# ndmarco/BayesFMMM

Hardware: AMD Instinct MI355X
Metric: Gibbs iterations/sec (whole node) at n_funct=4096, K=3, P=30 (higher is better)
Workload: dtype f64; 1 GPU; BFMMM_warm_start sweep, n_funct=4096, n_i=100, K=3, P=30, M=6, fp64, one independent chain per GPU (1 chain(s): a chain does not shard, replicas only); chains=1, chains_per_gpu=1

## Files before the change

bayesfmmm_amd/_lib.py:

```python
import ctypes as C
import os

_HERE = os.path.dirname(os.path.abspath(__file__))
LIB_PATH = os.environ.get("BFMMM_LIB_PATH", os.path.join(_HERE, "libbfmmm_hip.so"))

c_double_p = C.POINTER(C.c_double)
c_int64_p = C.POINTER(C.c_int64)


class BfmmmConfig(C.Structure):
    _fields_ = [("model", C.c_int32), ("n_funct", C.c_int32), ("K", C.c_int32), ("n_eigen", C.c_int32),
                ("basis_degree", C.c_int32), ("n_internal_knots", C.c_int32), ("P", C.c_int32),
                ("tot_mcmc_iters", C.c_int32), ("c", C.c_double * 8), ("b", C.c_double), ("nu_1", C.c_double),
                ("alpha1l", C.c_double), ("alpha2l", C.c_double), ("beta1l", C.c_double), ("beta2l", C.c_double),
                ("a_Z_PM", C.c_double), ("a_pi_PM", C.c_double), ("var_alpha3", C.c_double),
                ("var_epsilon1", C.c_double), ("var_epsilon2", C.c_double), ("alpha_nu", C.c_double),
                ("beta_nu", C.c_double), ("alpha_eta", C.c_double), ("beta_eta", C.c_double),
                ("alpha_0", C.c_double), ("beta_0", C.c_double)]


SYMBOLS = {
    "bfmmm_config_defaults": (None, [C.POINTER(BfmmmConfig)]),
    "bfmmm_create": (C.c_int, [C.POINTER(BfmmmConfig), C.c_int, c_double_p, c_double_p, c_int64_p, c_double_p,
                               c_double_p, C.POINTER(C.c_void_p)]),
    "bfmmm_destroy": (None, [C.c_void_p]),
    "bfmmm_create_batch": (C.c_int, [C.POINTER(BfmmmConfig), C.c_int, c_double_p, c_double_p, c_int64_p, c_double_p,
                                     c_double_p, C.c_int, C.POINTER(C.c_void_p)]),
    "bfmmm_create_from_basis_batch": (C.c_int, [C.POINTER(BfmmmConfig), C.c_int, c_double_p, c_double_p, c_int64_p, C.c_int,
                                                C.c_int, c_double_p, C.c_int, C.c_int, C.POINTER(C.c_void_p)]),
    "bfmmm_select_chain": (C.c_int, [C.c_void_p, C.c_int]),
    "bfmmm_n_chains": (C.c_int, [C.c_void_p]),
    "bfmmm_set_chain_id_stride": (C.c_int, [C.c_void_p, C.c_uint32]),
    "bfmmm_gather_best": (C.c_int, [C.POINTER(C.c_void_p), C.c_int, c_double_p, C.POINTER(C.c_int32), C.POINTER(C.c_int)]),
    "bfmmm_set_covariates": (C.c_int, [C.c_void_p, c_double_p, C.c_int, C.c_int]),
    "bfmmm_get_basis": (C.c_int, [C.c_void_p, c_double_p, C.c_int64]),
    "bfmmm_set_state": (C.c_int, [C.c_void_p, C.c_char_p, c_double_p, C.c_int64]),
    "bfmmm_get_state": (C.c_int, [C.c_void_p, C.c_char_p, c_double_p, C.c_int64]),
    "bfmmm_init_state": (C.c_int, [C.c_void_p, C.c_int, C.c_uint64, C.c_uint32]),
    "bfmmm_run": (C.c_int, [C.c_void_p, C.c_uint32, C.c_int, C.c_int, C.c_uint64, C.c_uint32, C.c_int, C.c_double]),
    "bfmmm_prepare_run": (C.c_int, [C.c_void_p, C.c_uint32, C.c_int, C.c_int, C.c_uint64, C.c_uint32, C.c_int]),
    "bfmmm_set_slot_base": (C.c_int, [C.c_void_p, C.c_int]),
    "bfmmm_create_from_basis": (C.c_int, [C.POINTER(BfmmmConfig), C.c_int, c_double_p, c_double_p, c_int64_p, C.c_int, C.c_int,
                                          c_double_p, C.c_int, C.POINTER(C.c_void_p)]),
    "bfmmm_tempered_transition": (C.c_int, [C.c_void_p, C.c_uint32, C.c_int, C.c_int, C.c_double, C.c_uint64, C.c_uint32,
                                            c_double_p, C.POINTER(C.c_int)]),
    "bfmmm_get_chain": (C.c_int, [C.c_void_p, C.c_char_p, C.c_int, c_double_p, C.c_int64]),
    "bfmmm_chain_diagnostics": (C.c_int, [C.c_void_p, C.c_char_p, C.c_int, C.c_int, C.c_int64, c_double_p, c_double_p, c_double_p,
                                          c_double_p, c_double_p, c_double_p, c_double_p, C.c_int64]),
    "bfmmm_debug_get": (C.c_int, [C.c_void_p, C.c_char_p, c_double_p, C.c_int64, c_int64_p]),
    "bfmmm_set_profile": (C.c_int, [C.c_void_p, C.c_int]),
    "bfmmm_get_timing": (C.c_int, [C.c_void_p, C.c_char_p, C.POINTER(C.c_double), c_int64_p]),
    "bfmmm_set_exact_instances": (None, [C.c_int]),
    "bfmmm_set_solo_pair_gram": (None, [C.c_int]),
    "bfmmm_last_error": (C.c_char_p, []),
}

_LIB = None


def load():
    global _LIB
    if _LIB is None:
        if not os.path.exists(LIB_PATH):
            raise RuntimeError(
                f"{LIB_PATH} is missing: build it with `python -c 'import __graft_entry__ as g; g.build()'` "
                "(hipcc --offload-arch=gfx950). bayesfmmm_amd has no CPU fallback.")
        lib = C.CDLL(LIB_PATH)
        for name, (res, args) in SYMBOLS.items():
            fn = getattr(lib, name)
            fn.restype = res
            fn.argtypes = args
        _LIB = lib
    return _LIB


class BfmmmError(RuntimeError):
    pass


def check(rc):
    if rc != 0:
        raise BfmmmError(load().bfmmm_last_error().decode())
```

bayesfmmm_amd/csrc/bfmmm_capi.hip:

```cpp
#include "../../include/bfmmm.h"
#include "model.hpp"
#include "rng.hpp"

#include <algorithm>
#include <cmath>
#include <cstdio>
#include <cstring>
#include <map>
#include <chrono>
#include <mutex>
#include <string>
#include <tuple>
#include <vector>

namespace bfmmm {
int launch_stats_functional(int degree, int n, int P, int LREC, const int64_t* off, const double* t, const double* y,
                            const double* knots, int n_knots, double* rec, int* ni, double* B_dense, int* err,
                            hipStream_t st);
void launch_stats_multivariate(int n, int P, int LREC, const double* Y, double* rec, int* ni, hipStream_t st);
void launch_stats_totals(int n, int LREC, int yy_off, const double* rec, const int* ni, double* out_yy,
                         long long* out_counts, hipStream_t st);
int launch_curve(const Ctx& c, int which, int do_update, hipStream_t st);
int curve_blocks(int n, int P);
void prepare_curve_kernels();
void prepare_sweep_kernels();
void launch_pair_gram(const Ctx& c, int do_pg, int NKS, int KS, hipStream_t st);
int pair_gram_body(const Ctx& c, int KS, int& G);
size_t pair_gram_lds_bytes(const Dims& d, int KS);
void launch_pg_reduce(const Ctx& c, int NKS, hipStream_t st);
bool pgp_geometry(const Dims& d, int nch, int KS, int NKS, PgPack& g);
size_t pgp_pack_doubles(const PgPack& g);
void launch_pair_gram_pack(const Ctx& c, const PgPack& g, double* pack, hipStream_t st);
void launch_factor(const Ctx& c, hipStream_t st);
int launch_sweep(const Ctx& c, hipStream_t st);
void launch_sweep_tables(const Ctx& c, hipStream_t st);
size_t sweep_tab_ints(int A);
void launch_loglik(const Ctx& c, int use_rss_part, int r_stored, hipStream_t st);
void launch_loglik_flush(const Ctx& c, hipStream_t st, uint32_t* status_out);
void launch_fill_slots(const Ctx& c, double* chain, const double* cur, size_t len, int s0, int s1, hipStream_t st);
void launch_cov_block(const Ctx& c, hipStream_t st);
int cov_step_blocks(int nblk_curve);
int cov_w2_chunks(int n);
void prepare_cov_kernels();
bool cov_block_fits(const Ctx& c);
#ifdef BFMMM_TIMELINE
void fetch_wgtrace(unsigned long long* out);
void fetch_ztrace(unsigned long long* out);
void fetch_zphase(unsigned long long* out);
void fetch_fct(unsigned long long* out);
#endif
}

using namespace bfmmm;

static thread_local std::string g_err;
static constexpr int GRAPH_UNROLL = 10;
static std::mutex g_capture_mutex;
static int fail(const std::string& msg) { g_err = msg; return 1; }

#define HIPCHK(x)                                                                                   \
// ... 10 lines not shown
enum { FAM_TOTAL = 0, FAM_Z, FAM_PG, FAM_FACTOR, FAM_SWEEP, FAM_CHI, FAM_LOGLIK, FAM_REDUCE, FAM_COUNT };
static const char* kFamNames[FAM_COUNT] = {"total", "curve_z", "pair_gram", "factor", "sweep", "curve_chi", "loglik", "pg_reduce"};

struct bfmmm_handle {
  bfmmm_config cfg;
  int device = 0;
  hipStream_t st = nullptr;
  hipEvent_t evA = nullptr;
  Ctx c;
  int nch = 1;
  int sel = 0;
  int T = 0;
  int64_t n_obs = 0;
  double* d_t = nullptr; double* d_y = nullptr; int64_t* d_off = nullptr; double* d_knots = nullptr; int n_knots = 0;
  std::vector<void*> allocs;
  char* arena = nullptr;
  char* arena_cov = nullptr;
  uint32_t* status_host = nullptr;
  uint32_t* status_dev = nullptr;
  size_t pg_part_doubles = 0;
  static constexpr int MAX_SUB = 4;
  char* dry_snap = nullptr;
  size_t dry_snap_bytes = 0;
  double* pg_pack[MAX_SUB + 1] = {};
  size_t pg_pack_doubles[MAX_SUB + 1] = {};
  hipStream_t sub_st[MAX_SUB] = {nullptr, nullptr, nullptr, nullptr};
  hipEvent_t sub_ev[MAX_SUB] = {nullptr, nullptr, nullptr, nullptr};
  struct CachedGraph { int sub, kind, reps; hipGraphExec_t g; };
  std::vector<CachedGraph> graphs;
  using GraphKey = std::tuple<uint32_t, int, uint64_t, uint32_t, int, int>;
  GraphKey g_key;
  bool g_valid = false;
  int last_md = -1;
  double last_route[5] = {0, 0, 0, -1, 0};
  int64_t tab_key = -1;
  int launch_error = 0;
  int slot_base = 0;
  double* tt_save = nullptr;
  std::vector<double> B_host;
  bool state_dirty = true;
  int profile = 0;
  double fam_ms[FAM_COUNT] = {0};
  int64_t fam_launches[FAM_COUNT] = {0};
  hipEvent_t ev0 = nullptr, ev1 = nullptr;
};

static hipError_t copy_sync(bfmmm_handle* h, void* dst, const void* src, size_t bytes, hipMemcpyKind kind) {
  hipError_t e = hipMemcpyAsync(dst, src, bytes, kind, h->st);
  if (e != hipSuccess) return e;
  return hipStreamSynchronize(h->st);
}

template <typename T>
static int dalloc(bfmmm_handle* h, T** p, size_t count) {
  void* q = nullptr;
  const size_t bytes = std::max<size_t>(count, 1) * sizeof(T);
  HIPCHK(hipMalloc(&q, bytes));
  HIPCHK(hipMemsetAsync(q, 0, bytes, h->st));
  h->allocs.push_back(q);
  *p = (T*)q;
  return 0;
}

static void drop_graphs(bfmmm_handle* h) {
  for (const auto& e : h->graphs) (void)hipGraphExecDestroy(e.g);
  h->graphs.clear();
  h->g_valid = false;
// ... 803 lines not shown
  if (!h) return fail("bfmmm_run: null handle");
  if (n_iters < 0 || first_iter < h->slot_base || first_iter - h->slot_base + n_iters > h->T)
    return fail("bfmmm_run: iterations exceed the allocated chain");
  HIPCHK(hipSetDevice(h->device));
  Ctx c = h->c;
  const int MD = phi_chi_zero ? 1 : (c.d.M + 1);
  set_md(c.d, MD);
  c.seed = seed; c.chain = chain; c.mask = mask;
  Plan plan = make_plan(mask, MD);
  if (c.d.D > 0) { plan.z = true; plan.chi = true; plan.use_rss_part = 1; }
  c.defer_loglik = (c.d.D == 0) ? 1 : 0;
  c.ll_use_part = plan.use_rss_part;
  h->last_md = MD;
  int nsub = 1;
  if (!h->profile && h->nch >= 4) nsub = 2;
  if (const char* env_split = h->profile ? nullptr : getenv("BFMMM_BATCH_SPLIT"))
    nsub = std::max(1, std::min({atoi(env_split), (int)bfmmm_handle::MAX_SUB, h->nch / 2}));
  Sub subs[bfmmm_handle::MAX_SUB];
  h->sub_st[0] = h->st;
  for (int q = 0, q0 = 0; q < nsub; ++q) {
    const int cnt = h->nch / nsub + (q < h->nch % nsub ? 1 : 0);
    if (pg_route(h, c.d, plan.pg, cnt, h->profile ? bfmmm_handle::MAX_SUB : q, subs[q].r)) return 1;
    if (!h->sub_st[q]) HIPCHK(hipStreamCreateWithFlags(&h->sub_st[q], hipStreamNonBlocking));
    if (!h->sub_ev[q]) HIPCHK(hipEventCreateWithFlags(&h->sub_ev[q], hipEventDisableTiming));
    subs[q].c = chain_ctx(c, (unsigned)q0);
    subs[q].c.nch = cnt;
    subs[q].st = h->sub_st[q];
    q0 += cnt;
  }
  {
    const PgRoute& r0 = subs[0].r;
    int G = 0;
    const int body = r0.packed ? -1 : pair_gram_body(subs[0].c, r0.KS, G);
    const double v[5] = {r0.packed ? 1.0 : 0.0, (double)r0.KS, (double)r0.NKS, (double)body, (double)G};
    memcpy(h->last_route, v, sizeof v);
  }
  c.defer_hyper = (c.defer_loglik && plan.pg && plan.chi && h->nch == 1 && !subs[0].r.packed && subs[0].r.NKS >= 2) ? 1 : 0;
  subs[0].c.defer_hyper = c.defer_hyper;
  if (!prepare_only) {
    ensure_sweep_tables(h, c, mask);
    hipLaunchKernelGGL(k_run_begin, dim3(h->nch), dim3(64), 0, h->st, h->c, (uint32_t)first_iter, (uint32_t)h->slot_base, tt_step, beta,
                       h->state_dirty ? 1 : 0);
    h->state_dirty = false;
    for (int f = 0; f < FAM_COUNT; ++f) { h->fam_ms[f] = 0; h->fam_launches[f] = 0; }
  }
  if (h->profile) {
    if (prepare_only) return 0;
    HIPCHK(hipEventRecord(h->ev0, h->st));
    if (run_profiled(h, c, plan, subs[0].r, n_iters, tt_step)) return 1;
    return finish_run(h, c, plan, mask, first_iter, n_iters, false);
  }
  const bool fuse = plan.z && plan.z_update && plan.chi && c.d.D == 0 && n_iters >= 2 && tt_step == 0;
  const bool defer = !fuse && plan.z && plan.z_update && plan.factor && (mask & U_Z) && c.d.D == 0 && c.d.K <= 4 && c.d.BW <= 5 &&
                     n_iters >= 2 && tt_step == 0;
  const bool bodies = fuse || defer;
  const int body_kind = fuse ? GK_FUSED : GK_DEFERRED;
  const int nrep = bodies ? n_iters - 1 : n_iters;
  const bool whole = bodies && nsub == 1 && n_iters <= WHOLE_MAX && c.defer_loglik && h->status_dev != nullptr;
  std::vector<std::pair<int, int>> segs;
  const int kind = bodies ? body_kind : GK_FULL;
  if (whole) {
    segs.push_back({GK_WHOLE, n_iters});
  } else {
    for (int q = 0; q < nrep / GRAPH_UNROLL; ++q) segs.push_back({kind, GRAPH_UNROLL});
    if (nrep % GRAPH_UNROLL) segs.push_back({kind, nrep % GRAPH_UNROLL});
    if (bodies) segs.push_back({GK_CLOSING, 1});
  }
  const bfmmm_handle::GraphKey key{mask, MD, seed, chain, nsub, (bfmmm::g_exact_instances ? 1 : 0) | (bfmmm::g_solo_pair_gram ? 2 : 0)};
  if (n_iters > 0 && !(h->g_valid && h->g_key == key)) { drop_graphs(h); h->g_key = key; h->g_valid = true; }
  std::vector<FreshGraph> fresh;
  std::vector<hipGraphExec_t> seq[bfmmm_handle::MAX_SUB];
  for (int s = 0; s < nsub; ++s)
    for (const auto& sg : segs) {
      hipGraphExec_t g = nullptr;
      if (cached_graph(h, s, sg.first, sg.second, subs[s].st, fresh, [&]() { queue_graph(h, c, subs[s], plan, sg.first, sg.second, body_kind); }, &g))
        return 1;
      seq[s].push_back(g);
    }
  if (prepare_only) return dry_launch(h, c, mask, subs, nsub, fresh, first_iter, tt_step, beta);
  HIPCHK(hipEventRecord(h->ev0, h->st));
  if (nsub > 1) HIPCHK(hipEventRecord(h->evA, h->st));
  for (int q = 1; q < nsub; ++q) HIPCHK(hipStreamWaitEvent(subs[q].st, h->evA, 0));
  for (int s = 0; s < nsub && n_iters > 0; ++s) {
    if (bodies && !whole) launch_curve(subs[s].c, 0, plan.z_update, subs[s].st);
    for (hipGraphExec_t g : seq[s]) HIPCHK(hipGraphLaunch(g, subs[s].st));
  }
  for (int q = 1; q < nsub; ++q) { HIPCHK(hipEventRecord(h->sub_ev[q], subs[q].st)); HIPCHK(hipStreamWaitEvent(h->st, h->sub_ev[q], 0)); }
  return finish_run(h, c, plan, mask, first_iter, n_iters, whole);
}

extern "C" int bfmmm_set_slot_base(bfmmm_handle* h, int base) {
  if (!h || base < 0) return fail("bfmmm_set_slot_base: bad arguments");
  h->slot_base = base;
  return 0;
}

extern "C" int bfmmm_run(bfmmm_handle* h, uint32_t mask, int first_iter, int n_iters, uint64_t seed, uint32_t chain,
                         int phi_chi_zero, double beta) {
  return run_impl(h, mask, first_iter, n_iters, seed, chain, phi_chi_zero, beta, 0);
}

// ... 199 lines not shown
  const std::string s(name);
  HIPCHK(hipStreamSynchronize(h->st));
  if (s == "dims") {
    const double v[] = {(double)d.n, (double)d.K, (double)d.P, (double)d.M, (double)d.BW, (double)d.LG, (double)d.LREC,
                        (double)d.MD, (double)d.A, (double)d.R, (double)d.NT, (double)d.n_obs_total, (double)d.half_sum, c.YY};
    const int64_t cnt = sizeof v / sizeof v[0];
    if (capacity < cnt) return fail("bfmmm_debug_get: buffer too small");
    memcpy(out, v, sizeof v);
    *count = cnt;
    return 0;
  }
  if (s == "pg_route") {
    const int64_t cnt = sizeof h->last_route / sizeof h->last_route[0];
    if (capacity < cnt) return fail("bfmmm_debug_get: buffer too small");
    memcpy(out, h->last_route, sizeof h->last_route);
    *count = cnt;
    return 0;
  }
  struct Arr { const char* nm; const double* p; int64_t len; };
  const Arr arrs[] = {{"rec", c.rec, (int64_t)d.n * d.LREC}, {"H", c.H, (int64_t)d.R * d.LG}, {"tvec", c.tvec, (int64_t)d.A * d.P},
                      {"H2", c.H2, (int64_t)d.R * d.P * (2 * d.BW + 2)},
                      {"Cmat", c.Cmat, (int64_t)d.A * d.P * d.P},
                      {"theta", c.theta, (int64_t)d.K * (d.M + 1) * d.P}};
  for (const Arr& a : arrs)
    if (s == a.nm) {
      if (capacity < a.len) return fail("bfmmm_debug_get(" + s + "): buffer too small");
      HIPCHK(copy_sync(h, out, a.p, sizeof(double) * (size_t)a.len, hipMemcpyDeviceToHost));
      *count = a.len;
      return 0;
    }
  return fail("bfmmm_debug_get: unknown name '" + s + "'");
}

namespace bfmmm { int g_exact_instances = 1; int g_solo_pair_gram = 1; }
extern "C" void bfmmm_set_exact_instances(int enable) { bfmmm::g_exact_instances = enable ? 1 : 0; }
extern "C" void bfmmm_set_solo_pair_gram(int enable) { bfmmm::g_solo_pair_gram = enable ? 1 : 0; }

extern "C" int bfmmm_set_profile(bfmmm_handle* h, int enable) {
  if (!h) return fail("bfmmm_set_profile: null handle");
  h->profile = enable ? 1 : 0;
  return 0;
}

extern "C" int bfmmm_get_timing(bfmmm_handle* h, const char* name, double* ms, int64_t* launches) {
  if (!h || !name || !ms || !launches) return fail("bfmmm_get_timing: null argument");
  for (int f = 0; f < FAM_COUNT; ++f)
    if (!strcmp(name, kFamNames[f])) { *ms = h->fam_ms[f]; *launches = h->fam_launches[f]; return 0; }
  return fail("bfmmm_get_timing: unknown name");
}

#include <rccl/rccl.h>

#define NCCLCHK(x)                                                                                   \
  do {                                                                                              \
    ncclResult_t r_ = (x);                                                                          \
    if (r_ != ncclSuccess) {                                                                        \
      char buf_[512];                                                                               \
      snprintf(buf_, sizeof buf_, "RCCL error %s at %s:%d (%s)", ncclGetErrorString(r_), __FILE__, __LINE__, #x); \
      return fail(buf_);                                                                            \
    }                                                                                               \
  } while (0)

struct GatherGuard {
  std::vector<ncclComm_t> comms;
  std::vector<int> devs;
  std::vector<double*> bufs;
  ~GatherGuard() {
    for (ncclComm_t cm : comms) if (cm) (void)ncclCommDestroy(cm);
    for (size_t i = 0; i < bufs.size(); ++i)
// ... 73 lines not shown
```

bayesfmmm_amd/csrc/kernels_sweep.hip:

```cpp
#include "model.hpp"
#include "rng.hpp"
#include "scalar_jobs.hpp"
#include "factor_core.hpp"
#include "z_proposal.hpp"

#include <algorithm>
#include <cstdlib>
#include <type_traits>

namespace bfmmm {



#ifdef BFMMM_TIMELINE
void fetch_fct(unsigned long long* out) { (void)hipMemcpyFromSymbol(out, HIP_SYMBOL(g_fct), sizeof(unsigned long long) * 8); }
#endif

__device__ inline void lds_barrier() { asm volatile("s_waitcnt lgkmcnt(0)\n\ts_barrier" ::: "memory"); }

#ifdef BFMMM_TIMELINE
__device__ unsigned long long g_wgtrace[3 * 1024];
void fetch_wgtrace(unsigned long long* out) { (void)hipMemcpyFromSymbol(out, HIP_SYMBOL(g_wgtrace), sizeof(unsigned long long) * 3 * 1024); }
#endif

// ... 107 lines not shown
  TSTAMP0(c, 41);
  lds_barrier();
  TSTAMP0(c, 42);
  constexpr int NW = PG_THREADS / 64;
  const int wave = tid >> 6, lane = tid & 63, lr = lane & 15, kq = lane >> 4;
  const int ntl = __builtin_amdgcn_readfirstlane(max(0, min(PGS_TMAX, (d.RT - wave + NW - 1) / NW)));
  int o1[PGS_TMAX], o2[PGS_TMAX];
#pragma unroll
  for (int q = 0; q < PGS_TMAX; ++q) {
    const int row = (wave + NW * q) * 16 + lr;
    o1[q] = o2[q] = NP;
    if (q < ntl && row < d.R) { const int zz = row / d.NCC; o1[q] = zz; o2[q] = NZZ + (row - zz * d.NCC); }
  }
  double4_t acc[PGS_TMAX];
#pragma unroll
  for (int q = 0; q < PGS_TMAX; ++q) acc[q] = double4_t{0.0, 0.0, 0.0, 0.0};
  switch (ntl) {
    case 1: pg_solo_tiles<1>(sP, sB, KSP, KQ, nchunk, o1, o2, lr, kq, acc); break;
    case 2: pg_solo_tiles<2>(sP, sB, KSP, KQ, nchunk, o1, o2, lr, kq, acc); break;
    case 3: pg_solo_tiles<3>(sP, sB, KSP, KQ, nchunk, o1, o2, lr, kq, acc); break;
    case 4: pg_solo_tiles<4>(sP, sB, KSP, KQ, nchunk, o1, o2, lr, kq, acc); break;
    default: break;
  }
#pragma unroll
  for (int q = 0; q < PGS_TMAX; ++q)
    if (q < ntl) {
      double* out = c0.pg_part + ((size_t)ks * d.NT + (size_t)(wave + NW * q) * d.CTG + ct) * 256 + lane;
      __builtin_nontemporal_store(acc[q][0], out); __builtin_nontemporal_store(acc[q][1], out + 64);
      __builtin_nontemporal_store(acc[q][2], out + 128); __builtin_nontemporal_store(acc[q][3], out + 192);
    }
  TSTAMP0(c, 44);
}

template <bool BATCH, bool GROUPS>
__global__ __launch_bounds__(PG_THREADS) void k_pair_gram(Ctx c0, int KS, int nks, int do_pg, int G) {
  const int nch = BATCH ? c0.nch : 1;
  TIMELINE(c0, 1);
#ifdef BFMMM_TIMELINE
  const int wgid = blockIdx.x + gridDim.x * blockIdx.y;
  if (threadIdx.x == 0 && wgid < 1024) {
    unsigned id, hw;
    asm volatile("s_getreg_b32 %0, hwreg(HW_REG_XCC_ID)" : "=s"(id));
    asm volatile("s_getreg_b32 %0, hwreg(HW_REG_HW_ID)" : "=s"(hw));
    g_wgtrace[3 * wgid] = wall_clock64();
    g_wgtrace[3 * wgid + 1] = ((unsigned long long)(id & 0xf) << 32) | hw;
  }
  struct EndTrace { int w; __device__ ~EndTrace() { if (threadIdx.x == 0 && w < 1024) g_wgtrace[3 * w + 2] = wall_clock64(); } } et_{wgid};
#endif
  extern __shared__ __attribute__((aligned(16))) double smem[];
  const Dims& d = c0.d;
  const int n = d.n, K = d.K, MD = d.MD;
  const int ks = blockIdx.y, ct = blockIdx.x;
  if (ct == d.CTG + 1) {
    if (ks < nch && threadIdx.x < 256) {
      const Ctx c = chain_ctx(c0, (unsigned)ks);
      job_pi_alpha(c);
      TSTAMP(c, 46);
    } else if (ks >= nch && ks < 2 * nch && threadIdx.x < 256) {
      const Ctx c = chain_ctx(c0, (unsigned)(ks - nch));
      if (c.dyn->hyper_pending) {
        job_hyper(c, false);
        __syncthreads();
        if (threadIdx.x == 0) c.dyn->hyper_pending = 0u;
      }
    }
    return;
  }
  if (ks >= nks) return;
  if (!do_pg) return;
  const bool single = ct == d.CTG;
  if constexpr (!BATCH) {
    if (do_pg == PG_SOLO && !single) { pg_solo_g(c0, KS, ks, ct, smem); return; }
  }
  const int ncol = single ? d.CTS * 16 : 16;
  const int col0 = single ? d.LG : ct * 16;
  const int colend = single ? d.LG + d.P : d.LG;
  const int i0 = ks * KS;
  const int RS = K + MD + 1, ONE = K;
  const int NP = d.NZZ + d.NCC, RP = NP + 1;
  const int KSP = KS + 2;
  const int KQ4 = KS >> 2;
  auto pos = [&](int il) { return (il & 3) * KQ4 + (il >> 2); };
  const int GG = GROUPS ? G : 1;
  const int TB = RS + (single ? 0 : RP);
  double* sB = smem;
  double* sW = sB + (size_t)ncol * KSP;
  double* sP = sW + (size_t)RS * KSP;
  const int tid = threadIdx.x;
  constexpr int UW = 12, UB = 6;
  const int ncw = K + MD - 1;
  const int nB = KS * ncol;
  auto loadW = [&](const double* Zq, const double* chiq, int il0, int cb, double (&v)[UW]) {
    const int i = min(i0 + il0 + tid, n - 1);
#pragma unroll
    for (int u = 0; u < UW; ++u) {
      const int col = min(cb + u, ncw - 1);
      v[u] = (col < K) ? Zq[i + (size_t)n * col] : chiq[i + (size_t)n * (col - K)];
    }
  };
  auto storeW = [&](int il0, int cb, const double (&v)[UW]) {
    const int il = il0 + tid;
    if (il >= KS) return;
    const bool live = i0 + il < n;
#pragma unroll
    for (int u = 0; u < UW; ++u) {
// ... 1588 lines not shown
    return;
  }
  if (c.dyn->ll_pending) deferred_loglik(c, red);
  if (status_out && threadIdx.x == 0) {
    __hip_atomic_store(&status_out[blockIdx.z], c.dyn->status, __ATOMIC_RELEASE, __HIP_MEMORY_SCOPE_SYSTEM);
  }
}

__global__ void k_fill_slots(double* chain, const double* cur, size_t len, int s0, int s1, size_t chain_bytes) {
  chain = ptr_shift(chain, blockIdx.z * chain_bytes);
  cur = ptr_shift(cur, blockIdx.z * chain_bytes);
  const size_t total = len * (size_t)(s1 - s0);
  for (size_t e = blockIdx.x * (size_t)blockDim.x + threadIdx.x; e < total; e += (size_t)gridDim.x * blockDim.x)
    chain[(size_t)s0 * len + e] = cur[e % len];
}

static size_t pair_gram_lds_bytes(const Dims& d, int KS, int G) {
  const int RS = d.K + d.MD + 1, RP = d.NZZ + d.NCC + 1;
  const size_t tables = (size_t)(KS + 2) * std::max(16 + G * (RS + RP), d.CTS * 16 + G * RS) + 128;
  return std::max(tables, (size_t)std::max(PI_ALPHA_LDS_DOUBLES, HYPER_LDS_DOUBLES)) * sizeof(double);
}
size_t pair_gram_lds_bytes(const Dims& d, int KS) { return pair_gram_lds_bytes(d, KS, 1); }

int pair_gram_body(const Ctx& c, int KS, int& G) {
  const Dims& d = c.d;
  const int ncw = d.K + d.MD - 1;
  G = 1;
  if (c.nch > 1 && d.D == 0 && d.RT < 8)
    while (G < c.nch && pair_gram_lds_bytes(d, KS, G + 1) <= 144 * 1024 && (size_t)(G + 1) * ncw * KS <= 12 * 512) ++G;
  if (c.nch > 1) return G > 1 ? 3 : 2;
  return (g_solo_pair_gram && pg_solo_fits(d, KS)) ? 1 : 0;
}

void launch_pair_gram(const Ctx& c, int do_pg, int NKS, int KS, hipStream_t st) {
  const Dims& d = c.d;
  int G = 1;
  const int body = pair_gram_body(c, KS, G);
  const size_t lds = pair_gram_lds_bytes(d, KS, G);
  if (body == 3) hipLaunchKernelGGL((k_pair_gram<true, true>), dim3(d.CTG + 2, do_pg ? std::max(NKS, c.nch) : c.nch, 1), dim3(PG_THREADS), lds, st, c, KS, NKS, do_pg, G);
  else if (body == 2) hipLaunchKernelGGL((k_pair_gram<true, false>), dim3(d.CTG + 2, do_pg ? std::max(NKS, c.nch) : c.nch, 1), dim3(PG_THREADS), lds, st, c, KS, NKS, do_pg, 1);
  else {
    const int pg = (do_pg && body == 1) ? PG_SOLO : do_pg;
    hipLaunchKernelGGL((k_pair_gram<false, false>), dim3(d.CTG + 2, do_pg ? NKS : 1, 1), dim3(PG_THREADS), lds, st, c, KS, NKS, pg, 1);
  }
}

size_t pgp_lds_bytes(const PgPack& g) {
  const size_t lg = 2 * (16 * (size_t)PGP_RB + (size_t)g.NQG * 16 * g.SLS), ls = 2 * (16 * (size_t)PGP_RB + (size_t)g.NQS * 16 * g.SLS);
  return std::max(lg, ls) * sizeof(double);
}
bool pgp_geometry(const Dims& d, int nch, int KS, int NKS, PgPack& g) {
  if (d.mv || d.D > 0 || d.K > 4 || d.MD - 1 > 8 || d.P > 32 || (d.LREC & 1) || (KS & 15)) return false;
  g.KS = KS; g.NKS = NKS;
  g.NP2 = (d.LG + 31) / 32;
  g.TG = (nch * d.R + 15) / 16; g.TS = (nch * d.A + 15) / 16;
  g.WPG = PGP_WPG;
  g.NRG = (g.TG + PGP_WPG - 1) / PGP_WPG; g.NCG = (g.NP2 + 1) / 2; g.NWG_S = (g.TS + PGP_WPG - 1) / PGP_WPG;
  g.SLG = (d.NZZ + d.NCC + 1 + 1) & ~1; g.SLS = (d.K + d.MD + 1 + 1) & ~1;
  g.NQG = std::min(nch, (PGP_WPG * 16 + d.R - 2) / d.R + 1); g.NQS = std::min(nch, (PGP_WPG * 16 + d.A - 2) / d.A + 1);
  g.NTP = g.TG * 2 * g.NP2 + g.TS * 2;
  const int NV = d.K + d.MD - 1;
  if (std::max(g.NQG, g.NQS) * NV * 16 > PGP_NWV * 64 * PGP_WPG) return false;
  return pgp_lds_bytes(g) <= 64 * 1024;
}
size_t pgp_pack_doubles(const PgPack& g) { return (size_t)g.NKS * g.NTP * 256; }

void launch_pair_gram_pack(const Ctx& c, const PgPack& g, double* pack, hipStream_t st) {
  const dim3 grid(g.NRG * g.NCG + g.NWG_S, g.NKS, 1);
  hipLaunchKernelGGL(k_pair_gram_pack<PGP_WPG>, grid, dim3(64 * PGP_WPG), pgp_lds_bytes(g), st, c, g, pack);
  const int nblk_red = (g.NTP * 256 * 4 + 255) / 256;
  hipLaunchKernelGGL(k_pg_reduce_pack, dim3(nblk_red), dim3(256), 0, st, c, g, pack);
}

void launch_pg_reduce(const Ctx& c, int NKS, hipStream_t st) {
  const int nthreads = c.d.NT * 256 * 4;
  hipLaunchKernelGGL(k_pg_reduce, dim3((nthreads + 255) / 256, 1, c.nch), dim3(256), 0, st, c, NKS);
// ... 108 lines not shown
```

bayesfmmm_amd/csrc/model.hpp:

```cpp
#pragma once
#include <hip/hip_runtime.h>
#include <stdint.h>

namespace bfmmm {

constexpr int KMAX = 8;
constexpr int PMAX = 64;
constexpr int BWMAX = 5;
constexpr int BWWIDE = 31;
constexpr int BWMID = 15;

enum : uint32_t {
  U_Z = 1u << 0, U_PI = 1u << 1, U_ALPHA3 = 1u << 2, U_PHI = 1u << 3, U_DELTA = 1u << 4, U_A = 1u << 5,
  U_GAMMA = 1u << 6, U_NU = 1u << 7, U_TAU = 1u << 8, U_SIGMA = 1u << 9, U_CHI = 1u << 10,
  U_ETA = 1u << 11, U_TAU_ETA = 1u << 12, U_XI = 1u << 13, U_DELTA_XI = 1u << 14, U_A_XI = 1u << 15,
  U_GAMMA_XI = 1u << 16, U_LOGLIK = 1u << 17
};

struct Hyper {
  double c[KMAX];
  double b, nu_1;
  double alpha1l, alpha2l, beta1l, beta2l;
  double a_Z_PM, a_pi_PM, var_alpha3, var_epsilon1, var_epsilon2;
  double alpha_nu, beta_nu, alpha_eta, beta_eta, alpha_0, beta_0;
// ... 168 lines not shown
  int NP2;
};

#define BFMMM_CHAIN_PTRS(X_)                                                                                         \
  X_(dyn) X_(Z) X_(chi) X_(theta) X_(delta) X_(Aa) X_(gamma) X_(logz_part) X_(rss_part) X_(pg_part) X_(H) X_(H2)       \
  X_(tvec) X_(rvec) X_(hq) X_(Lz) X_(gstd) X_(zprep) X_(chi_norm) X_(piprep) X_(Cmat)                        \
  X_(c_nu) X_(c_chi) X_(c_Z) X_(c_pi) X_(c_alpha3) X_(c_delta) X_(c_A) X_(c_sigma) X_(c_tau) X_(c_gamma) X_(c_Phi) X_(c_loglik)
#define BFMMM_CHAIN_PTRS_COV(X_)                                                                                     \
  X_(thetaX) X_(tau_eta) X_(gamma_xi) X_(delta_xi) X_(A_xi) X_(stil) X_(yyp_part) X_(cfull) X_(gfull) X_(w2_part)      \
  X_(H2aa) X_(gstd2) X_(Wdir) X_(C2) X_(Lz2) X_(step_part) X_(thetaN) X_(delta_cur)                                   \
  X_(c_eta) X_(c_xi) X_(c_tau_eta) X_(c_gamma_xi) X_(c_delta_xi) X_(c_A_xi)

template <typename T>
__host__ __device__ inline T* ptr_shift(T* p, size_t bytes) { return (T*)((char*)p + bytes); }

__host__ __device__ inline Ctx chain_ctx(const Ctx& c0, unsigned q) {
  Ctx c = c0;
  const size_t o1 = (size_t)q * c0.chain_bytes, o2 = (size_t)q * c0.chain_bytes_cov;
#define X_(f) c.f = ptr_shift(c0.f, o1);
  BFMMM_CHAIN_PTRS(X_)
#undef X_
#define X_(f) c.f = ptr_shift(c0.f, o2);
  BFMMM_CHAIN_PTRS_COV(X_)
#undef X_
  c.chain = c0.chain + q * c0.chain_id_stride;
  return c;
}
#ifdef __HIPCC__
__device__ inline Ctx chain_view(const Ctx& c0) { return chain_ctx(c0, blockIdx.z); }
#endif

extern int g_exact_instances;
extern int g_solo_pair_gram;

__host__ __device__ inline int tri_index(int n, int a, int b) {
  return a * n - (a * (a - 1)) / 2 + (b - a);
}

#ifdef BFMMM_TIMELINE
struct Timeline {
  unsigned long long* s; int k;
  __device__ Timeline(const Ctx& c, int k_) : s(c.dyn->stamps), k(k_) {
    if (blockIdx.x == 0 && blockIdx.y == 0 && threadIdx.x == 0) s[2 * k] = wall_clock64();
    if (threadIdx.x == 0) atomicMax(&s[16 + k], (unsigned long long)wall_clock64());
  }
  __device__ ~Timeline() { if (threadIdx.x == 0) atomicMax(&s[2 * k + 1], (unsigned long long)wall_clock64()); }
};
#define TIMELINE(c, k) Timeline tl_((c), (k))
#define TSTAMP(c, i) do { if (threadIdx.x == 0) atomicMax(&(c).dyn->stamps[i], (unsigned long long)wall_clock64()); } while (0)
#define TSTAMP0(c, i) do { if (threadIdx.x == 0 && blockIdx.x == 0 && blockIdx.y == 0) (c).dyn->stamps[i] = wall_clock64(); } while (0)
#else
#define TIMELINE(c, k) do { } while (0)
#define TSTAMP(c, i) do { } while (0)
#define TSTAMP0(c, i) do { } while (0)
#endif

template <int CTRL>
__device__ inline double dpp_add(double v) {
  const int lo = __builtin_amdgcn_update_dpp(0, __double2loint(v), CTRL, 0xf, 0xf, true);
  const int hi = __builtin_amdgcn_update_dpp(0, __double2hiint(v), CTRL, 0xf, 0xf, true);
  return v + __hiloint2double(hi, lo);
}
__device__ inline double row16_sum(double v) {
  v = dpp_add<0xB1>(v);
  v = dpp_add<0x4E>(v);
  v = dpp_add<0x141>(v);
// ... 35 lines not shown
```

bayesfmmm_amd/csrc/scalar_jobs.hpp:

```cpp
#pragma once
#include "model.hpp"
#include "rng.hpp"

namespace bfmmm {

__device__ inline double block_sum256(double v, double* scratch) {
  __syncthreads();
  scratch[threadIdx.x] = v;
  __syncthreads();
  for (int o = 128; o > 0; o >>= 1) {
    if ((int)threadIdx.x < o) scratch[threadIdx.x] += scratch[threadIdx.x + o];
    __syncthreads();
  }
  const double r = scratch[0];
  __syncthreads();
  return r;
}

__device__ inline double logGamma_ref(double x) { return log(tgamma(x)); }

__device__ inline void deferred_loglik(const Ctx& c, double* red) {
  Dyn* dyn = c.dyn;
  const int tid = threadIdx.x;
  double rss = dyn->rss;
// ... 53 lines not shown
    const bool is_sum = tid >= 6 * K;
    const int row = is_sum ? tid - 6 * K : tid / K, k = is_sum ? 0 : tid - row * K;
    const double sc = (row < 2) ? c.h.a_pi_PM : ((row < 4) ? alpha3 : a3_ph);
    double arg = 0.0;
#pragma unroll
    for (int k2 = 0; k2 < KMAX; ++k2)
      if (k2 < K) {
        const double term = sc * ((row & 1) ? pi_new[k2] : pi_old[k2]);
        if (is_sum) arg += term;
        else if (k2 == k) arg = term;
      }
    t.lg[tid] = lgamma_pos(arg);
  } else if (tid >= 64 && tid < 64 + 2 * K) {
    const int e = tid - 64;
    double arg = 1.0;
#pragma unroll
    for (int k = 0; k < KMAX; ++k) { if (k < K && e == k) arg = pi_old[k]; if (k < K && e == K + k) arg = pi_new[k]; }
    t.lp[e] = log(arg);
  } else if (tid == 128 || tid == 129) {
    t.dt[tid - 128] = (tid == 128) ? dtruncnorm_lo_log(a3_ph, a3_ph, sd, 0.0) : dtruncnorm_lo_log(alpha3, alpha3, sd, 0.0);
  }
  __syncthreads();
}

__device__ inline void job_pi_prepare(const Ctx& c) {
  extern __shared__ __attribute__((aligned(16))) double smem[];
  Dyn* dyn = c.dyn;
  const PiAlphaTabs t = pi_alpha_layout(smem);
  pi_alpha_tables(c, make_key(c.seed, c.chain, dyn->iter + 1u, 0u), t);
  for (int e = threadIdx.x; e < PI_TAB_DOUBLES; e += 256) c.piprep[e] = smem[e];
  if (threadIdx.x == 0) { dyn->piprep_iter = dyn->iter + 1u; dyn->zprep_chain = c.chain; dyn->zprep_seed = c.seed; dyn->piprep_valid = 1u; }
}

__device__ inline void job_pi_alpha(const Ctx& c) {
  extern __shared__ __attribute__((aligned(16))) double smem[];
  double (*red)[256] = (double (*)[256])smem;
  double* S = smem + KMAX * 256;
  const PiAlphaTabs t = pi_alpha_layout(S + KMAX);
  double *g = t.g, *lg = t.lg, *ph_s = t.ph_s, *lu = t.lu, *lp = t.lp, *dt = t.dt;
  const Dims& d = c.d;
  const int K = d.K, n = d.n, tid = threadIdx.x;
  Dyn* dyn = c.dyn;
  const uint32_t mask = c.mask;
  if (dyn->ll_pending) deferred_loglik(c, smem);
  if (!(mask & (U_PI | U_ALPHA3))) {
    if (tid == 0) {
      c.c_alpha3[dyn->slot] = dyn->alpha3;
      for (int k = 0; k < K; ++k) c.c_pi[(size_t)dyn->slot * K + k] = dyn->pi[k];
    }
    return;
  }
  const bool pre = dyn->piprep_valid && dyn->piprep_iter == dyn->iter && dyn->tt_step == 0 &&
                   dyn->zprep_chain == c.chain && dyn->zprep_seed == c.seed;
  if (pre) {
    for (int e = tid; e < PI_TAB_DOUBLES; e += 256) t.g[e] = c.piprep[e];
  } else {
    pi_alpha_tables(c, make_key(c.seed, c.chain, dyn->iter, dyn->tt_step), t);
  }
  {
    double acc[KMAX];
#pragma unroll
    for (int k = 0; k < KMAX; ++k) acc[k] = 0.0;
    const int per = (c.nblk_curve + 255) / 256;
    for (int b = tid * per; b < min(c.nblk_curve, (tid + 1) * per); ++b)
#pragma unroll
      for (int k = 0; k < KMAX; ++k)
        if (k < K) acc[k] += c.logz_part[(size_t)b * K + k];
#pragma unroll
    for (int k = 0; k < KMAX; ++k) red[k][tid] = acc[k];
    __syncthreads();
    for (int o = 128; o > 0; o >>= 1) {
      if (tid < o)
#pragma unroll
        for (int k = 0; k < KMAX; ++k)
          if (k < K) red[k][tid] += red[k][tid + o];
      __syncthreads();
    }
// ... 382 lines not shown
```

include/bfmmm.h:

```cpp
#ifndef BFMMM_H
#define BFMMM_H

#include <stdint.h>

#ifdef __cplusplus
extern "C" {
#endif

typedef struct bfmmm_handle bfmmm_handle;

enum { BFMMM_MODEL_FUNCTIONAL = 0, BFMMM_MODEL_MULTIVARIATE = 1 };

enum {
  BFMMM_U_Z = 1 << 0, BFMMM_U_PI = 1 << 1, BFMMM_U_ALPHA3 = 1 << 2, BFMMM_U_PHI = 1 << 3,
  BFMMM_U_DELTA = 1 << 4, BFMMM_U_A = 1 << 5, BFMMM_U_GAMMA = 1 << 6, BFMMM_U_NU = 1 << 7,
  BFMMM_U_TAU = 1 << 8, BFMMM_U_SIGMA = 1 << 9, BFMMM_U_CHI = 1 << 10,
  BFMMM_U_ETA = 1 << 11, BFMMM_U_TAU_ETA = 1 << 12, BFMMM_U_XI = 1 << 13, BFMMM_U_DELTA_XI = 1 << 14,
  BFMMM_U_A_XI = 1 << 15, BFMMM_U_GAMMA_XI = 1 << 16, BFMMM_U_LOGLIK = 1 << 17
};
#define BFMMM_SWEEP_NU_Z  (BFMMM_U_Z | BFMMM_U_PI | BFMMM_U_ALPHA3 | BFMMM_U_NU | BFMMM_U_TAU | BFMMM_U_SIGMA | BFMMM_U_LOGLIK)
#define BFMMM_SWEEP_THETA (BFMMM_U_PHI | BFMMM_U_DELTA | BFMMM_U_A | BFMMM_U_GAMMA | BFMMM_U_TAU | BFMMM_U_SIGMA | BFMMM_U_CHI | BFMMM_U_LOGLIK)
#define BFMMM_SWEEP_WARM  (BFMMM_SWEEP_NU_Z | BFMMM_SWEEP_THETA)
#define BFMMM_COV_MEAN (BFMMM_U_ETA | BFMMM_U_TAU_ETA)
#define BFMMM_COV_XI   (BFMMM_U_XI | BFMMM_U_DELTA_XI | BFMMM_U_A_XI | BFMMM_U_GAMMA_XI)
// ... 38 lines not shown
int bfmmm_get_basis(bfmmm_handle* h, double* out, int64_t capacity);

int bfmmm_set_state(bfmmm_handle* h, const char* name, const double* values, int64_t count);
int bfmmm_get_state(bfmmm_handle* h, const char* name, double* out, int64_t capacity);

int bfmmm_init_state(bfmmm_handle* h, int stage, uint64_t seed, uint32_t chain);

int bfmmm_run(bfmmm_handle* h, uint32_t mask, int first_iter, int n_iters, uint64_t seed, uint32_t chain,
              int phi_chi_zero, double beta);

int bfmmm_prepare_run(bfmmm_handle* h, uint32_t mask, int first_iter, int n_iters, uint64_t seed, uint32_t chain,
                      int phi_chi_zero);

int bfmmm_set_slot_base(bfmmm_handle* h, int base);

int bfmmm_tempered_transition(bfmmm_handle* h, uint32_t mask, int iter, int N_t, double beta_N_t, uint64_t seed,
                              uint32_t chain, double* logA, int* accepted);

int bfmmm_get_chain(bfmmm_handle* h, const char* name, int n_slots, double* out, int64_t capacity);

int bfmmm_chain_diagnostics(bfmmm_handle* h, const char* name, int first_slot, int n_slots, int64_t max_workspace_bytes,
                            double* rhat, double* ess_bulk, double* ess_tail, double* ess_mean, double* mcse_mean,
                            double* mean, double* sd, int64_t capacity);

int bfmmm_debug_get(bfmmm_handle* h, const char* name, double* out, int64_t capacity, int64_t* count);

int bfmmm_set_profile(bfmmm_handle* h, int enable);
int bfmmm_get_timing(bfmmm_handle* h, const char* name, double* ms, int64_t* launches);

void bfmmm_set_exact_instances(int enable);

void bfmmm_set_solo_pair_gram(int enable);

const char* bfmmm_last_error(void);

#ifdef __cplusplus
}
#endif
#endif
```

Measured before the change: 18480 Gibbs iterations/sec.

## Add MFMA solo path for single-column pair-gram tail and split deferred loglik

In the solo pair-gram kernel, the 'single' column tile blocks now run a dedicated MFMA f64 path (pg_solo_s) that stages Z*chi products and basis columns in LDS, instead of the generic path. The deferred loglik work also moves off the pi/alpha scalar job into its own block of the extra grid column, so the two can run in parallel. The aim is to shorten the critical path of the pair-gram launch. The cost is extra LDS sizing, more code paths and a new toggle that is part of the graph key.

```diff
diff --git a/bayesfmmm_amd/_lib.py b/bayesfmmm_amd/_lib.py
--- a/bayesfmmm_amd/_lib.py
+++ b/bayesfmmm_amd/_lib.py
@@ -52,6 +52,7 @@
     "bfmmm_get_timing": (C.c_int, [C.c_void_p, C.c_char_p, C.POINTER(C.c_double), c_int64_p]),
     "bfmmm_set_exact_instances": (None, [C.c_int]),
     "bfmmm_set_solo_pair_gram": (None, [C.c_int]),
+    "bfmmm_set_solo_pair_gram_tail": (None, [C.c_int]),
     "bfmmm_last_error": (C.c_char_p, []),
 }
 
diff --git a/bayesfmmm_amd/csrc/bfmmm_capi.hip b/bayesfmmm_amd/csrc/bfmmm_capi.hip
--- a/bayesfmmm_amd/csrc/bfmmm_capi.hip
+++ b/bayesfmmm_amd/csrc/bfmmm_capi.hip
@@ -26,6 +26,7 @@
 void prepare_sweep_kernels();
 void launch_pair_gram(const Ctx& c, int do_pg, int NKS, int KS, hipStream_t st);
 int pair_gram_body(const Ctx& c, int KS, int& G);
+int pair_gram_tail(const Ctx& c, int KS, int NKS, int body);
 size_t pair_gram_lds_bytes(const Dims& d, int KS);
 void launch_pg_reduce(const Ctx& c, int NKS, hipStream_t st);
 bool pgp_geometry(const Dims& d, int nch, int KS, int NKS, PgPack& g);
@@ -102,7 +103,7 @@
   GraphKey g_key;
   bool g_valid = false;
   int last_md = -1;
-  double last_route[5] = {0, 0, 0, -1, 0};
+  double last_route[6] = {0, 0, 0, -1, 0, 0};
   int64_t tab_key = -1;
   int launch_error = 0;
   int slot_base = 0;
@@ -972,7 +973,8 @@
     const PgRoute& r0 = subs[0].r;
     int G = 0;
     const int body = r0.packed ? -1 : pair_gram_body(subs[0].c, r0.KS, G);
-    const double v[5] = {r0.packed ? 1.0 : 0.0, (double)r0.KS, (double)r0.NKS, (double)body, (double)G};
+    const int tail = (r0.packed || !plan.pg) ? 0 : pair_gram_tail(subs[0].c, r0.KS, r0.NKS, body);
+    const double v[6] = {r0.packed ? 1.0 : 0.0, (double)r0.KS, (double)r0.NKS, (double)body, (double)G, (double)tail};
     memcpy(h->last_route, v, sizeof v);
   }
   c.defer_hyper = (c.defer_loglik && plan.pg && plan.chi && h->nch == 1 && !subs[0].r.packed && subs[0].r.NKS >= 2) ? 1 : 0;
@@ -1006,7 +1008,8 @@
     if (nrep % GRAPH_UNROLL) segs.push_back({kind, nrep % GRAPH_UNROLL});
     if (bodies) segs.push_back({GK_CLOSING, 1});
   }
-  const bfmmm_handle::GraphKey key{mask, MD, seed, chain, nsub, (bfmmm::g_exact_instances ? 1 : 0) | (bfmmm::g_solo_pair_gram ? 2 : 0)};
+  const bfmmm_handle::GraphKey key{mask, MD, seed, chain, nsub, (bfmmm::g_exact_instances ? 1 : 0) | (bfmmm::g_solo_pair_gram ? 2 : 0) |
+                                                                        (bfmmm::g_solo_pair_gram_tail ? 4 : 0)};
   if (n_iters > 0 && !(h->g_valid && h->g_key == key)) { drop_graphs(h); h->g_key = key; h->g_valid = true; }
   std::vector<FreshGraph> fresh;
   std::vector<hipGraphExec_t> seq[bfmmm_handle::MAX_SUB];
@@ -1272,9 +1275,10 @@
   return fail("bfmmm_debug_get: unknown name '" + s + "'");
 }
 
-namespace bfmmm { int g_exact_instances = 1; int g_solo_pair_gram = 1; }
+namespace bfmmm { int g_exact_instances = 1; int g_solo_pair_gram = 1; int g_solo_pair_gram_tail = 1; }
 extern "C" void bfmmm_set_exact_instances(int enable) { bfmmm::g_exact_instances = enable ? 1 : 0; }
 extern "C" void bfmmm_set_solo_pair_gram(int enable) { bfmmm::g_solo_pair_gram = enable ? 1 : 0; }
+extern "C" void bfmmm_set_solo_pair_gram_tail(int enable) { bfmmm::g_solo_pair_gram_tail = enable ? 1 : 0; }
 
 extern "C" int bfmmm_set_profile(bfmmm_handle* h, int enable) {
   if (!h) return fail("bfmmm_set_profile: null handle");
diff --git a/bayesfmmm_amd/csrc/kernels_sweep.hip b/bayesfmmm_amd/csrc/kernels_sweep.hip
--- a/bayesfmmm_amd/csrc/kernels_sweep.hip
+++ b/bayesfmmm_amd/csrc/kernels_sweep.hip
@@ -163,6 +163,87 @@
   TSTAMP0(c, 44);
 }
 
+constexpr int PG_SOLO_S = 4;
+constexpr int PG_SOLO_LL = 8;
+constexpr int PGS_SU = PGS_KS / (PG_THREADS / 32);
+
+__device__ inline void pg_solo_s(const Ctx& c0, int KS, int ks, double* smem) {
+  const Dims& d = c0.d;
+  const int n = d.n, K = d.K, MD = d.MD, tid = threadIdx.x;
+  const int i0 = ks * KS;
+  const int nlive = min(KS, n - i0);
+  const int nchunk = (nlive + 15) >> 4;
+  const int nst = nchunk * 16;
+  const int KSP = KS + 2, KQ = KS >> 2;
+  const int ncol = d.CTS * 16;
+  double* sB = smem;
+  double* sS = sB + ncol * KSP;
+  const bool wl = tid < nlive;
+  const int iw = i0 + tid;
+  double z[4], x[8];
+#pragma unroll
+  for (int a = 0; a < 4; ++a) z[a] = (wl && a < K) ? c0.Z[iw + (size_t)n * a] : 0.0;
+#pragma unroll
+  for (int m = 0; m < 8; ++m) x[m] = (wl && m < MD - 1) ? c0.chi[iw + (size_t)n * m] : 0.0;
+  const int sh = (d.CTS == 1) ? 4 : 5;
+  const int cc = tid & (ncol - 1), ilg = tid >> sh, ilstep = PG_THREADS >> sh;
+  const bool colok = cc < d.P;
+  const double* src = c0.rec + (size_t)i0 * d.LREC + min(d.LG + cc, d.LREC - 1);
+  double vb[PGS_SU];
+#pragma unroll
+  for (int u = 0; u < PGS_SU; ++u) {
+    const int il = ilg + ilstep * u;
+    vb[u] = (il < nlive && colok) ? src[(size_t)il * d.LREC] : 0.0;
+  }
+  if (tid < nst) {
+    double* dst = sS + (tid & 3) * KQ + (tid >> 2);
+    const double xt[9] = {1.0, x[0], x[1], x[2], x[3], x[4], x[5], x[6], x[7]};
+#pragma unroll
+    for (int a = 0; a < 4; ++a)
+#pragma unroll
+      for (int m = 0; m < 9; ++m)
+        if (a < K && m < MD) dst[(a * MD + m) * KSP] = z[a] * xt[m];
+    dst[d.A * KSP] = 0.0;
+  }
+#pragma unroll
+  for (int u = 0; u < PGS_SU; ++u) {
+    const int il = ilg + ilstep * u;
+    if (il < nst) sB[cc * KSP + (il & 3) * KQ + (il >> 2)] = vb[u];
+  }
+  lds_barrier();
+  const int wave = __builtin_amdgcn_readfirstlane(tid >> 6), lane = tid & 63, lr = lane & 15, kq = lane >> 4;
+  if (wave >= d.AT * d.CTS) return;
+  const int at = wave / d.CTS, cs = wave - at * d.CTS;
+  const int row = at * 16 + lr;
+  const v2d* pa = (const v2d*)(sS + (row < d.A ? row : d.A) * KSP + kq * KQ);
+  const v2d* pc = (const v2d*)(sB + (cs * 16 + lr) * KSP + kq * KQ);
+  struct Ops { v2d a[2], c[2]; };
+  auto load = [&](Ops& o, int t) { o.a[0] = pa[2 * t]; o.c[0] = pc[2 * t]; o.a[1] = pa[2 * t + 1]; o.c[1] = pc[2 * t + 1]; };
+  double4_t acc = double4_t{0.0, 0.0, 0.0, 0.0};
+  auto mfma = [&](const Ops& o) {
+#pragma unroll
+    for (int u = 0; u < 2; ++u) {
+      acc = __builtin_amdgcn_mfma_f64_16x16x4f64(o.a[u].x, o.c[u].x, acc, 0, 0, 0);
+      acc = __builtin_amdgcn_mfma_f64_16x16x4f64(o.a[u].y, o.c[u].y, acc, 0, 0, 0);
+    }
+  };
+  Ops s0, s1;
+  load(s0, 0);
+  for (int t = 0; t < nchunk; t += 2) {
+    if (t + 1 < nchunk) load(s1, t + 1);
+    __builtin_amdgcn_sched_barrier(0);
+    mfma(s0);
+    __builtin_amdgcn_sched_barrier(0);
+    if (t + 2 < nchunk) load(s0, t + 2);
+    __builtin_amdgcn_sched_barrier(0);
+    if (t + 1 < nchunk) mfma(s1);
+    __builtin_amdgcn_sched_barrier(0);
+  }
+  double* out = c0.pg_part + ((size_t)ks * d.NT + (size_t)d.RT * d.CTG + wave) * 256 + lane;
+  __builtin_nontemporal_store(acc[0], out); __builtin_nontemporal_store(acc[1], out + 64);
+  __builtin_nontemporal_store(acc[2], out + 128); __builtin_nontemporal_store(acc[3], out + 192);
+}
+
 template <bool BATCH, bool GROUPS>
 __global__ __launch_bounds__(PG_THREADS) void k_pair_gram(Ctx c0, int KS, int nks, int do_pg, int G) {
   const int nch = BATCH ? c0.nch : 1;
@@ -185,7 +266,7 @@
   if (ct == d.CTG + 1) {
     if (ks < nch && threadIdx.x < 256) {
       const Ctx c = chain_ctx(c0, (unsigned)ks);
-      job_pi_alpha(c);
+      job_pi_alpha(c, BATCH || !(do_pg & PG_SOLO_LL));
       TSTAMP(c, 46);
     } else if (ks >= nch && ks < 2 * nch && threadIdx.x < 256) {
       const Ctx c = chain_ctx(c0, (unsigned)(ks - nch));
@@ -194,6 +275,8 @@
         __syncthreads();
         if (threadIdx.x == 0) c.dyn->hyper_pending = 0u;
       }
+    } else if (!BATCH && (do_pg & PG_SOLO_LL) && ks == 2 * nch && threadIdx.x < 256) {
+      if (c0.dyn->ll_pending) deferred_loglik(c0, smem);
     }
     return;
   }
@@ -201,7 +284,8 @@
   if (!do_pg) return;
   const bool single = ct == d.CTG;
   if constexpr (!BATCH) {
-    if (do_pg == PG_SOLO && !single) { pg_solo_g(c0, KS, ks, ct, smem); return; }
+    if ((do_pg & PG_SOLO) && !single) { pg_solo_g(c0, KS, ks, ct, smem); return; }
+    if ((do_pg & PG_SOLO_S) && single) { pg_solo_s(c0, KS, ks, smem); return; }
   }
   const int ncol = single ? d.CTS * 16 : 16;
   const int col0 = single ? d.LG : ct * 16;
@@ -1856,6 +1940,14 @@
   return (g_solo_pair_gram && pg_solo_fits(d, KS)) ? 1 : 0;
 }
 
+int pair_gram_tail(const Ctx& c, int KS, int NKS, int body) {
+  if (body != 1 || !g_solo_pair_gram_tail) return 0;
+  int f = 0;
+  if (c.d.AT * c.d.CTS <= PG_THREADS / 64 && c.d.CTS <= 2) f |= PG_SOLO_S;
+  if (c.defer_loglik && NKS >= 3) f |= PG_SOLO_LL;
+  return f;
+}
+
 void launch_pair_gram(const Ctx& c, int do_pg, int NKS, int KS, hipStream_t st) {
   const Dims& d = c.d;
   int G = 1;
@@ -1864,8 +1956,9 @@
   if (body == 3) hipLaunchKernelGGL((k_pair_gram<true, true>), dim3(d.CTG + 2, do_pg ? std::max(NKS, c.nch) : c.nch, 1), dim3(PG_THREADS), lds, st, c, KS, NKS, do_pg, G);
   else if (body == 2) hipLaunchKernelGGL((k_pair_gram<true, false>), dim3(d.CTG + 2, do_pg ? std::max(NKS, c.nch) : c.nch, 1), dim3(PG_THREADS), lds, st, c, KS, NKS, do_pg, 1);
   else {
-    const int pg = (do_pg && body == 1) ? PG_SOLO : do_pg;
-    hipLaunchKernelGGL((k_pair_gram<false, false>), dim3(d.CTG + 2, do_pg ? NKS : 1, 1), dim3(PG_THREADS), lds, st, c, KS, NKS, pg, 1);
+    const int pg = (do_pg && body == 1) ? (PG_SOLO | pair_gram_tail(c, KS, NKS, body)) : do_pg;
+    const size_t lds1 = (pg & PG_SOLO_S) ? std::max(lds, (size_t)(KS + 2) * (d.CTS * 16 + d.A + 1) * sizeof(double)) : lds;
+    hipLaunchKernelGGL((k_pair_gram<false, false>), dim3(d.CTG + 2, do_pg ? NKS : 1, 1), dim3(PG_THREADS), lds1, st, c, KS, NKS, pg, 1);
   }
 }
 
diff --git a/bayesfmmm_amd/csrc/model.hpp b/bayesfmmm_amd/csrc/model.hpp
--- a/bayesfmmm_amd/csrc/model.hpp
+++ b/bayesfmmm_amd/csrc/model.hpp
@@ -224,6 +224,7 @@
 
 extern int g_exact_instances;
 extern int g_solo_pair_gram;
+extern int g_solo_pair_gram_tail;
 
 __host__ __device__ inline int tri_index(int n, int a, int b) {
   return a * n - (a * (a - 1)) / 2 + (b - a);
diff --git a/bayesfmmm_amd/csrc/scalar_jobs.hpp b/bayesfmmm_amd/csrc/scalar_jobs.hpp
--- a/bayesfmmm_amd/csrc/scalar_jobs.hpp
+++ b/bayesfmmm_amd/csrc/scalar_jobs.hpp
@@ -109,7 +109,7 @@
   if (threadIdx.x == 0) { dyn->piprep_iter = dyn->iter + 1u; dyn->zprep_chain = c.chain; dyn->zprep_seed = c.seed; dyn->piprep_valid = 1u; }
 }
 
-__device__ inline void job_pi_alpha(const Ctx& c) {
+__device__ inline void job_pi_alpha(const Ctx& c, bool loglik = true) {
   extern __shared__ __attribute__((aligned(16))) double smem[];
   double (*red)[256] = (double (*)[256])smem;
   double* S = smem + KMAX * 256;
@@ -119,7 +119,7 @@
   const int K = d.K, n = d.n, tid = threadIdx.x;
   Dyn* dyn = c.dyn;
   const uint32_t mask = c.mask;
-  if (dyn->ll_pending) deferred_loglik(c, smem);
+  if (loglik && dyn->ll_pending) deferred_loglik(c, smem);
   if (!(mask & (U_PI | U_ALPHA3))) {
     if (tid == 0) {
       c.c_alpha3[dyn->slot] = dyn->alpha3;
diff --git a/include/bfmmm.h b/include/bfmmm.h
--- a/include/bfmmm.h
+++ b/include/bfmmm.h
@@ -94,6 +94,8 @@
 
 void bfmmm_set_solo_pair_gram(int enable);
 
+void bfmmm_set_solo_pair_gram_tail(int enable);
+
 const char* bfmmm_last_error(void);
 
 #ifdef __cplusplus
```

Measured after the change: 18800 Gibbs iterations/sec, median of 6. 1.7% higher.
